# bot15498/Lisec

Hardware: AMD Instinct MI355X
Metric: lyft_samples_per_sec_fwd_bwd (higher is better)
Workload: dtype f32; 1 GPU; Lyft grid 8x200x400x35, U20K synthetic cloud, 1 sample/GPU/step, voxelise+VFE+3xConv3D+RPN fwd+bwd, MSE+MSE, SGD-Nesterov; global_batch=1, parallelism=dp1, launch=step plan (lisec_step_plan_run: 196 recorded launches / event edges per step), voxels=9424

## Files before the change

include/lisec_hip.h:

```cpp
#ifndef LISEC_HIP_H
#define LISEC_HIP_H

#include <stddef.h>
#include <stdint.h>

#ifdef __cplusplus
extern "C" {
#endif

#define LISEC_OK 0
#define LISEC_EINVAL (-1)
#define LISEC_ENOSPC (-2)
#define LISEC_EHIP (-3)

typedef void* lisec_stream_t;

const char* lisec_last_error(void);
int lisec_abi_version(void);
int lisec_device_info(char* name, int cap);

typedef struct {
    double xSize, ySize, zSize;
    int maxVoxelX, maxVoxelY, maxVoxelZ;
    int sampleSize;
// ... 273 lines not shown

int lisec_bn_backward_apply_coef(const float* dA, int da_stride, const float* y, const float* bnstate, long long M, int C,
                                 int relu, const float* coef, float* dy, lisec_stream_t stream);

typedef struct lisec_copy_desc {
    const float* src;
    float* dst;
    int rows, cols;
    long long src_stride, dst_stride;
} lisec_copy_desc;
int lisec_copy2d_batched(const lisec_copy_desc* device_table, int n, lisec_stream_t stream);

int lisec_fold_depth(const float* in, float* out, int D, long long HW, int C, int inverse, const float* mask,
                     lisec_stream_t stream);

int lisec_relu_mask(float* grad, const float* act, long long n, lisec_stream_t stream);

int lisec_colsum(const float* x, int stride, long long M, int C, float* out, void* workspace,
                 size_t workspace_bytes, lisec_stream_t stream);

int lisec_rpn_loss(const float* head, const float* y_cls, const float* y_reg, long long M, int kind,
                   float grad_scale, float* dhead, float* loss_out, void* workspace, size_t workspace_bytes,
                   lisec_stream_t stream);

int lisec_rpn_loss_eval(const float* head, const float* y_cls, const float* y_reg, long long M, int kind, double* acc,
                        void* workspace, size_t workspace_bytes, lisec_stream_t stream);

#define LISEC_LOSS_MAX_METRICS 4
enum {
    LISEC_LOSS_MSE = 0,
    LISEC_LOSS_MAE = 1,
    LISEC_LOSS_MAPE = 2,
    LISEC_LOSS_MSLE = 3,
    LISEC_LOSS_HUBER = 4,
    LISEC_LOSS_LOGCOSH = 5,
    LISEC_LOSS_BCE = 6,
    LISEC_LOSS_POISSON = 7,
    LISEC_LOSS_SIGMOID_CE_CLAMPED = 8,
    LISEC_LOSS_SMOOTH_L1 = 9,
    LISEC_METRIC_BINARY_ACCURACY = 10,
    LISEC_METRIC_CATEGORICAL_ACCURACY = 11
};
typedef struct lisec_loss_term {
    int kind;
    int from_logits;
    float param;
// ... 286 lines not shown
```

lisec_amd/_lib.py:

```python
import ctypes
import os
from ctypes import POINTER, Structure, c_char_p, c_double, c_float, c_int, c_int32, c_size_t, c_void_p

_HERE = os.path.dirname(os.path.abspath(__file__))
LIB_PATH = os.path.join(_HERE, "liblisec_hip.so")


class LisecError(RuntimeError):
    pass


class VoxelCfg(Structure):
    _fields_ = [("xSize", c_double), ("ySize", c_double), ("zSize", c_double),
                ("maxVoxelX", c_int), ("maxVoxelY", c_int), ("maxVoxelZ", c_int),
                ("sampleSize", c_int)]


class VfeParams(Structure):
    _fields_ = [("kernel", c_void_p * 3), ("gamma", c_void_p * 3), ("beta", c_void_p * 3),
                ("moving_mean", c_void_p * 3), ("moving_var", c_void_p * 3)]


class VfeGrads(Structure):
    _fields_ = [("kernel", c_void_p * 3), ("gamma", c_void_p * 3), ("beta", c_void_p * 3)]
# ... 263 lines not shown
    lib.lisec_bn_backward_apply_coef.argtypes = [P, c_int, P, P, LL, c_int, c_int, P, P, P]
    lib.lisec_conv_forward_masked.restype = c_int
    lib.lisec_conv_forward_masked.argtypes = [POINTER(ConvGeom), P, P, P, P, c_int, P, P, P, P, c_size_t, P, P, c_int, P]
    lib.lisec_conv_forward_workspace_bytes.restype = c_size_t
    lib.lisec_conv_forward_workspace_bytes.argtypes = [POINTER(ConvGeom)]
    lib.lisec_conv_forward_rows_workspace_bytes.restype = c_size_t
    lib.lisec_conv_forward_rows_workspace_bytes.argtypes = [POINTER(ConvGeom), c_int]
    lib.lisec_conv_wgrad_workspace_bytes.restype = c_size_t
    lib.lisec_conv_wgrad_workspace_bytes.argtypes = [POINTER(ConvGeom), c_int]
    lib.lisec_conv_wgrad.restype = c_int
    lib.lisec_conv_wgrad.argtypes = [POINTER(ConvGeom), P, P, c_int, P, P, P, c_size_t, c_int, P, P, P, c_int, P]
    lib.lisec_eltwise_workspace_bytes.restype = c_size_t
    lib.lisec_eltwise_workspace_bytes.argtypes = []
    lib.lisec_bn_backward.restype = c_int
    lib.lisec_bn_backward.argtypes = [P, c_int, P, P, LL, c_int, c_int, P, P, P, P, P, c_size_t, P]
    lib.lisec_relu_mask.restype = c_int
    lib.lisec_relu_mask.argtypes = [P, P, LL, P]
    lib.lisec_colsum.restype = c_int
    lib.lisec_colsum.argtypes = [P, c_int, LL, c_int, P, P, c_size_t, P]
    lib.lisec_rpn_loss.restype = c_int
    lib.lisec_rpn_loss.argtypes = [P, P, P, LL, c_int, c_float, P, P, P, c_size_t, P]
    lib.lisec_rpn_loss_eval.restype = c_int
    lib.lisec_rpn_loss_eval.argtypes = [P, P, P, LL, c_int, P, P, c_size_t, P]
    lib.lisec_head_loss.restype = c_int
    lib.lisec_head_loss.argtypes = [POINTER(LossCfg), P, P, P, LL, c_float, P, P, P, P, c_size_t, P]
    lib.lisec_head_loss_eval.restype = c_int
    lib.lisec_head_loss_eval.argtypes = [POINTER(LossCfg), P, P, P, LL, P, P, c_size_t, P]
    lib.lisec_head_loss_workspace_bytes.restype = c_size_t
    lib.lisec_head_loss_workspace_bytes.argtypes = []
    lib.lisec_detection_loss.restype = c_int
    lib.lisec_detection_loss.argtypes = [POINTER(DetectionLossCfg), P, P, P, LL, c_float, P, P, P, P, c_size_t, P]
    lib.lisec_detection_loss_eval.restype = c_int
    lib.lisec_detection_loss_eval.argtypes = [POINTER(DetectionLossCfg), P, P, P, LL, P, P, c_size_t, P]
    lib.lisec_detection_loss_workspace_bytes.restype = c_size_t
    lib.lisec_detection_loss_workspace_bytes.argtypes = []
    lib.lisec_detection_metrics.restype = c_int
    lib.lisec_detection_metrics.argtypes = [POINTER(DetectionMetricsCfg), P, P, P, LL, P, c_int, P, c_size_t, P]
    lib.lisec_detection_metrics_workspace_bytes.restype = c_size_t
    lib.lisec_detection_metrics_workspace_bytes.argtypes = []
    lib.lisec_sgd_nesterov_step.restype = c_int
    lib.lisec_sgd_nesterov_step.argtypes = [P, P, P, LL, c_float, c_float, P]
    lib.lisec_sgd_nesterov_step_dev.restype = c_int
    lib.lisec_sgd_nesterov_step_dev.argtypes = [P, P, P, LL, c_double, c_double, c_float, P, P]
    lib.lisec_sgd_nesterov_step_dev_part.restype = c_int
    lib.lisec_sgd_nesterov_step_dev_part.argtypes = [P, P, P, LL, c_double, c_double, c_float, P, P]
    lib.lisec_sgd_step_dev.restype = c_int
# ... 296 lines not shown
```

lisec_amd/csrc/common.h:

```cpp
#pragma once
#include <hip/hip_runtime.h>
#include <cstdarg>
#include <cstdio>
#include <cstdint>
#include <functional>
#include <tuple>
#include <utility>

#include "../../include/lisec_hip.h"

namespace lisec {

constexpr int kWave = 64;

void set_error(const char* fmt, ...);
const lisec_tuning& tuning();
int cu_count();

#define LISEC_CHECK_ARG(cond, ...)                 \
    do {                                           \
        if (!(cond)) {                             \
            ::lisec::set_error(__VA_ARGS__);       \
            return LISEC_EINVAL;                   \
        }                                          \
// ... 79 lines not shown
__device__ __forceinline__ T wave_sum(T v) {
#pragma unroll
    for (int o = 32; o > 0; o >>= 1) v += __shfl_xor(v, o, 64);
    return v;
}
template <typename T>
__device__ __forceinline__ T wave_max(T v) {
#pragma unroll
    for (int o = 32; o > 0; o >>= 1) {
        T u = __shfl_xor(v, o, 64);
        v = u > v ? u : v;
    }
    return v;
}
template <typename T>
__device__ __forceinline__ T wave_min(T v) {
#pragma unroll
    for (int o = 32; o > 0; o >>= 1) {
        T u = __shfl_xor(v, o, 64);
        v = u < v ? u : v;
    }
    return v;
}
#endif

}
```

lisec_amd/csrc/eltwise.hip:

```cpp
#include "bn.h"

namespace lisec {
namespace {

constexpr int kEwBlocks = 1024;
constexpr int kEwThreads = 256;

template <bool RELU>
__global__ void __launch_bounds__(kEwThreads)
k_bn_bwd_reduce(const float* __restrict__ dA, int da_stride, const float* __restrict__ y,
                const float* __restrict__ st, long long M, int C, double* __restrict__ parts) {
    __shared__ float red[2][kEwThreads][4];
    const int cq = C / 4;
    const int q = threadIdx.x % cq, rsub = threadIdx.x / cq, rows_per_iter = kEwThreads / cq;
    const float4 sc = reinterpret_cast<const float4*>(st)[q];
    const float4 sh = reinterpret_cast<const float4*>(st + C)[q];
    const float4 mu = reinterpret_cast<const float4*>(st + 2 * C)[q];
    const float4 is = reinterpret_cast<const float4*>(st + 3 * C)[q];
    float4 s1 = make_float4(0, 0, 0, 0), s2 = make_float4(0, 0, 0, 0);
    for (long long r = (long long)blockIdx.x * rows_per_iter + rsub; r < M; r += (long long)gridDim.x * rows_per_iter) {
        const float4 g = *reinterpret_cast<const float4*>(dA + r * da_stride + q * 4);
        const float4 v = *reinterpret_cast<const float4*>(y + r * C + q * 4);
#define LISEC_ACC(f)                                                         \
        {                                                                    \
// ... 66 lines not shown
        reinterpret_cast<float4*>(g)[i] = a;
    }
}

__global__ void __launch_bounds__(kEwThreads)
k_colsum(const float* __restrict__ x, int stride, long long M, int C, double* __restrict__ parts) {
    __shared__ float red[kEwThreads];
    const int cols = C < kEwThreads ? C : kEwThreads;
    const int c0 = blockIdx.y * kEwThreads;
    const int c = threadIdx.x % cols, rsub = threadIdx.x / cols, rows_per_iter = kEwThreads / cols;
    float s = 0.f;
    if (rsub < rows_per_iter)
        for (long long r = (long long)blockIdx.x * rows_per_iter + rsub; r < M; r += (long long)gridDim.x * rows_per_iter)
            s += x[r * stride + c0 + c];
    red[threadIdx.x] = rsub < rows_per_iter ? s : 0.f;
    __syncthreads();
    if (threadIdx.x < cols) {
        double a = 0.0;
        for (int k = 0; k < rows_per_iter; ++k) a += (double)red[k * cols + threadIdx.x];
        parts[(size_t)blockIdx.x * C + c0 + threadIdx.x] = a;
    }
}

__global__ void __launch_bounds__(kEwThreads)
k_loss(const float* __restrict__ head, const float* __restrict__ ycls, const float* __restrict__ yreg,
       long long M, int kind, float gscale, float* __restrict__ dhead, double* __restrict__ parts) {
    __shared__ double red[2][kEwThreads / 64];
    double lc = 0.0, lr = 0.0;
    const float wc = gscale / (float)(M * 2), wr = gscale / (float)(M * 14);
    for (long long i = blockIdx.x * (long long)kEwThreads + threadIdx.x; i < M * 16; i += (long long)gridDim.x * kEwThreads) {
        const long long m = i >> 4;
        const int c = (int)(i & 15);
        const float p = head[i];
        float g;
        if (c < 2) {
            const float t = ycls[m * 2 + c];
            if (kind == 0) {
                const float d = p - t;
                lc += (double)d * d;
                g = 2.f * d * wc;
            } else {
                const float tt = fminf(fmaxf(t, 0.f), 1.f);
                lc += (double)(fmaxf(p, 0.f) - p * tt + log1pf(expf(-fabsf(p))));
                g = (1.f / (1.f + expf(-p)) - tt) * wc;
            }
        } else {
            const float t = yreg[m * 14 + (c - 2)];
            const float d = p - t;
            if (kind == 0) {
                lr += (double)d * d;
                g = 2.f * d * wr;
            } else {
                const float ad = fabsf(d);
                lr += (double)(ad < 1.f ? 0.5f * d * d : ad - 0.5f);
                g = (ad < 1.f ? d : (d > 0.f ? 1.f : -1.f)) * wr;
            }
        }
        dhead[i] = g;
    }
    lc = wave_sum(lc); lr = wave_sum(lr);
    if (lane_id() == 0) { red[0][threadIdx.x >> 6] = lc; red[1][threadIdx.x >> 6] = lr; }
    __syncthreads();
    if (threadIdx.x < 2) {
        double a = 0.0;
        for (int k = 0; k < kEwThreads / 64; ++k) a += red[threadIdx.x][k];
        parts[(size_t)blockIdx.x * 2 + threadIdx.x] = a;
    }
}

__global__ void __launch_bounds__(256)
k_loss_finalize(const double* __restrict__ parts, int nparts, double M, float* __restrict__ out) {
    __shared__ double red[2][256];
    double a = 0.0, b = 0.0;
    for (int k = threadIdx.x; k < nparts; k += 256) { a += parts[2 * k]; b += parts[2 * k + 1]; }
    red[0][threadIdx.x] = a; red[1][threadIdx.x] = b;
    __syncthreads();
    for (int o = 128; o > 0; o >>= 1) {
        if ((int)threadIdx.x < o) { red[0][threadIdx.x] += red[0][threadIdx.x + o]; red[1][threadIdx.x] += red[1][threadIdx.x + o]; }
        __syncthreads();
    }
    if (threadIdx.x == 0) {
        a = red[0][0] / (M * 2.0); b = red[1][0] / (M * 14.0);
        out[0] = (float)(a + b); out[1] = (float)a; out[2] = (float)b;
    }
}

__global__ void __launch_bounds__(kEwThreads)
k_loss_eval(const float* __restrict__ head, const float* __restrict__ ycls, const float* __restrict__ yreg,
            long long M, int kind, double* __restrict__ parts) {
    __shared__ double red[2][kEwThreads / 64];
// ... 248 lines not shown
    LISEC_LAUNCH(k_colsum, dim3(nb, slabs), dim3(kEwThreads), 0, st, x, stride, M, C, parts);
    LISEC_LAUNCH_CHECK();
    return launch_reduce_parts(parts, nb, C, 1.0, out, nullptr, st);
}

extern "C" int lisec_rpn_loss(const float* head, const float* y_cls, const float* y_reg, long long M, int kind,
                              float grad_scale, float* dhead, float* loss_out, void* workspace,
                              size_t workspace_bytes, lisec_stream_t stream_) {
    LISEC_CHECK_ARG(head && y_cls && y_reg && dhead && loss_out && workspace && M > 0, "NULL pointer");
    LISEC_CHECK_ARG(kind == 0 || kind == 1, "loss kind must be 0 (mse+mse) or 1 (sigmoid-CE + SmoothL1)");
    if (workspace_bytes < lisec_eltwise_workspace_bytes()) {
        set_error("eltwise workspace too small");
        return LISEC_ENOSPC;
    }
    hipStream_t st = static_cast<hipStream_t>(stream_);
    double* parts = static_cast<double*>(workspace);
    int nb = ew_blocks(M * 16);
    LISEC_LAUNCH(k_loss, dim3(nb), dim3(kEwThreads), 0, st, head, y_cls, y_reg, M, kind, grad_scale, dhead, parts);
    LISEC_LAUNCH(k_loss_finalize, dim3(1), dim3(256), 0, st, parts, nb, (double)M, loss_out);
    LISEC_LAUNCH_CHECK();
    return LISEC_OK;
}

extern "C" int lisec_rpn_loss_eval(const float* head, const float* y_cls, const float* y_reg, long long M, int kind,
                                   double* acc, void* workspace, size_t workspace_bytes, lisec_stream_t stream_) {
    LISEC_CHECK_ARG(head && y_cls && y_reg && acc && workspace && M > 0, "NULL pointer");
    LISEC_CHECK_ARG(kind == 0 || kind == 1, "loss kind must be 0 (mse+mse) or 1 (sigmoid-CE + SmoothL1)");
    if (workspace_bytes < lisec_eltwise_workspace_bytes()) {
        set_error("eltwise workspace too small");
        return LISEC_ENOSPC;
    }
    hipStream_t st = static_cast<hipStream_t>(stream_);
    double* parts = static_cast<double*>(workspace);
    int nb = ew_blocks(M * 16);
    LISEC_LAUNCH(k_loss_eval, dim3(nb), dim3(kEwThreads), 0, st, head, y_cls, y_reg, M, kind, parts);
    LISEC_LAUNCH(k_loss_eval_finalize, dim3(1), dim3(256), 0, st, parts, nb, (double)M, acc);
    LISEC_LAUNCH_CHECK();
    return LISEC_OK;
}

extern "C" int lisec_sgd_nesterov_step(float* theta, const float* grad, float* velocity, long long n,
                                       float lr_t, float momentum, lisec_stream_t stream_) {
    LISEC_CHECK_ARG(theta && grad && velocity && n >= 0 && n % 4 == 0, "sgd: n must be a multiple of 4");
    if (n == 0) return LISEC_OK;
    LISEC_LAUNCH(k_sgd_nesterov, dim3(ew_blocks(n / 4)), dim3(kEwThreads), 0, static_cast<hipStream_t>(stream_),
                       theta, grad, velocity, n / 4, lr_t, momentum);
// ... 41 lines not shown
```

lisec_amd/csrc/head_fused.hip:

```cpp
#include "common.h"

namespace lisec {
namespace {

constexpr int kHeadCols = 16;
constexpr int kMaxUp = 512;

constexpr int kPairs = 16, kSlices = 16;
__global__ void __launch_bounds__(256)
k_head_compose(const float* __restrict__ up_kernel, const float* __restrict__ up_bias, const float* __restrict__ head_w,
               int taps, int Cin, int Cup, long long ts, long long cs, float* __restrict__ Wc,
               const float* __restrict__ bias_in, float* __restrict__ bias_out) {
    __shared__ float sH[kMaxUp * kHeadCols];
    __shared__ float red[kSlices][kPairs][kHeadCols + 1];
    for (int i = threadIdx.x; i < Cup * kHeadCols; i += 256) sH[i] = head_w[i];
    __syncthreads();
    const int pl = threadIdx.x & (kPairs - 1), q = threadIdx.x / kPairs;
    const int idx = blockIdx.x * kPairs + pl;
    const bool live = idx < taps * Cin;
    const int tap = live ? idx / Cin : 0, c = live ? idx - tap * Cin : 0;
    float acc[kHeadCols];
#pragma unroll
    for (int j = 0; j < kHeadCols; ++j) acc[j] = 0.f;
    const float* w = up_kernel + (size_t)tap * Cup * Cin + c;
// ... 75 lines not shown
            for (int j = 0; j < kHeadCols; ++j) red[threadIdx.x][j] += red[threadIdx.x + half][j];
        }
        __syncthreads();
    }
    if (threadIdx.x < kHeadCols)
        d_head_w[(size_t)n * kHeadCols + threadIdx.x] = fmaf(up_bias ? up_bias[n] : 0.f, S[threadIdx.x], red[0][threadIdx.x]);
    if (threadIdx.x == 0 && d_up_bias) {
        float b = 0.f;
        for (int j = 0; j < kHeadCols; ++j) b = fmaf(S[j], head_w[(size_t)n * kHeadCols + j], b);
        d_up_bias[n] = b;
    }
}

struct ShuffleBranches { int n; int ps[4]; float* T[4]; };
template <bool BACKWARD>
__global__ void __launch_bounds__(256)
k_head_shuffle(float* __restrict__ head, int Ho, int Wo, ShuffleBranches br) {
    const int i4 = blockIdx.x * 256 + threadIdx.x;
    if (i4 >= Ho * Wo * (kHeadCols / 4)) return;
    const int m = i4 >> 2, q = i4 & 3;
    const int h = m / Wo, w = m - h * Wo;
    float4 v = *reinterpret_cast<const float4*>(head + (size_t)i4 * 4);
    for (int b = 0; b < br.n; ++b) {
        const int ps = br.ps[b];
        const int pos = (h / ps) * (Wo / ps) + w / ps, tap = (h % ps) * ps + w % ps;
        float4* t = reinterpret_cast<float4*>(br.T[b] + ((size_t)pos * ps * ps + tap) * kHeadCols) + q;
        if (BACKWARD) *t = v;
        else { const float4 u = *t; v.x += u.x; v.y += u.y; v.z += u.z; v.w += u.w; }
    }
    if (!BACKWARD) *reinterpret_cast<float4*>(head + (size_t)i4 * 4) = v;
}

}
}

using namespace lisec;

extern "C" int lisec_head_compose(const float* up_kernel, const float* up_bias, const float* head_w, int taps, int Cin,
                                  int Cup, long long out_tap_stride, long long out_c_stride, float* Wc,
                                  const float* bias_in, float* bias_out, lisec_stream_t stream) {
    LISEC_CHECK_ARG(up_kernel && head_w && Wc && taps > 0 && Cin > 0 && Cup > 0 && Cup <= kMaxUp, "bad compose arguments");
    LISEC_CHECK_ARG(!bias_out || up_bias, "a composite bias needs the branch bias");
    LISEC_LAUNCH(k_head_compose, dim3(cdiv((long long)taps * Cin, kPairs)), dim3(256), 0, static_cast<hipStream_t>(stream),
                       up_kernel, up_bias, head_w, taps, Cin, Cup, out_tap_stride, out_c_stride, Wc, bias_in, bias_out);
    LISEC_LAUNCH_CHECK();
    return LISEC_OK;
}

extern "C" int lisec_head_compose_backward(const float* G, long long g_tap_stride, long long g_c_stride,
// ... 31 lines not shown
```

lisec_amd/network.py:

```python
import ctypes
import json
import os

import numpy as np
import torch

from . import _lib, lr_schedules, ops, optimizer_table
from .losses import DetectionLossSpec, LossSpec
from .params import DECONVS, MID, RPN_BLOCKS, ParamStore, fold_depth
from .vfe import VFEStack


LEGACY_LOSS_KINDS = {"mse": 0, "smoothl1_ce": 1}


def loss_acc_len(loss):
    if isinstance(loss, LossSpec):
        return 4 + loss.n_metrics
    if isinstance(loss, DetectionLossSpec):
        return 4 + 2 * loss.n_metrics
    LEGACY_LOSS_KINDS[loss]
    return 4


# ... 185 lines not shown
    def deconv_wgrad(self, L):
        net, a, p, G = self.net, self.net.act, self.net.params, self.net.grad
        c = L["conv"]
        if net.compose_head:
            b, (ts, cs) = L["slot"], L["wc_strides"]
            ops.conv_wgrad(c.g, a[L["src"]], self.branch_dy(L), L["G"], net.wgrad_ws, in_bn=net.bnstate[c.in_bn],
                           flags=ops.IN_RELU)
            ops.head_compose_backward(L["G"], ts, cs, p.view(L["up_kernel"]), p.view(L["up_bias"]),
                                      net.head_w[256 * b:256 * (b + 1)],
                                      net.head_db, L["k"] * L["k"], L["cin"], 256, p.grad_view(G, L["up_kernel"]),
                                      p.grad_view(G, L["up_bias"]), net.head_dw[256 * b:256 * (b + 1)])
            self.branches_left -= 1
            if self.branches_left == 0:
                net._head_split.run()
            return
        dy = self.branch_dy(L)
        if "wgeom" in L:
            ops.conv_wgrad(L["wgeom"], dy, a[L["src"]], p.grad_view(G, c.wname), net.wgrad_ws,
                           flags=ops.DY_RELU, dy_bn=net.bnstate[c.in_bn])
        else:
            ops.conv_wgrad(c.g, a[L["src"]], dy, p.grad_view(G, c.wname), net.wgrad_ws,
                           in_bn=net.bnstate[c.in_bn], flags=ops.IN_RELU, transpose_out=True)

    def heads(self):
        net, q, a, d = self.net, self.q, self.net.act, self.net.dact
        M = net.Ho * net.Wo
        if net.compose_head:
            net._dshuffle.run(d["head"], backward=True)
            q.defer(lambda: ops.colsum(d["head"], 16, M, 16, net.head_db, ws_tag="side"))
            return

        def head_leaves():
            ops.conv_wgrad(net.head_geom, a["concat"], d["head"], net.head_dw, net.wgrad_ws)
            ops.colsum(d["head"], 16, M, 16, net.head_db, ws_tag="side")
            net._head_split.run()

        def concat_leaves():
            ops.colsum(d["concat"], 768, M, 768, net.up_db, ws_tag="side")
            net._up_bias_split.run()

        q.run(head_leaves)
        ops.conv_forward(net.head_dgeom, d["head"], net.packed_t["head"][0], d["concat"])
        q.run(concat_leaves)

    def early_branches(self):
        net, q = self.net, self.q
        for L in net.layers:
            if L["kind"] == "deconv" and L["slot"] < len(DECONVS) - 1:
                ev = net._event("bwd_branch%d" % L["slot"])

                def branch(L=L, ev=ev):
# ... 244 lines not shown
        self.head_w = torch.empty(768, 16, dtype=f32, device=dev)
        self.head_b = torch.empty(16, dtype=f32, device=dev)
        self.fused_bias = torch.empty(16, dtype=f32, device=dev)
        if self.compose_head:
            self._shuffle = ops.HeadShuffle(Ho, Wo, [(L["T"], L["s"]) for L in self.layers
                                                     if L["kind"] == "deconv" and L["T"] is not None])
        self.parts = torch.empty(max_parts, dtype=torch.float64, device=dev)
        self._sinks, self._bsinks = {}, {}
        self.side = torch.cuda.Stream(device=dev, priority=0)
        self.side_queue = _SideQueue(self, None, self.side)

        self._tail_ok = {}
        self._loss_descs = {}
        self._early = None
        self.dense_dw_slabs = {}
        self._fwd_events = {}
        self._pack_pending = self._late_pending = False
        self._pack_done = self._pack_late = None
        self._packed_version = -1
        self.params_version = 0
        self.state_version = 0
        self._folded = {}
        self._train_ready = False
        self._iter_dev = torch.zeros(2, dtype=torch.int64, device=dev)
        self._iterations = 0
        self.momentum_cache = torch.ones(1, dtype=torch.float32, device=dev)
        self._lr_dev = torch.zeros(ctypes.sizeof(_lib.LrSchedule), dtype=torch.uint8, device=dev)
        self._lr_host = None
        self.loss_out = torch.zeros(3, dtype=f32, device=dev)
        self.metric_out = torch.zeros(2 * _lib.LOSS_MAX_METRICS, dtype=f32, device=dev)
        self.loss_counts = torch.zeros(2, dtype=torch.int64, device=dev)
        self.metric_pairs = torch.zeros(2 * _lib.DET_MAX_METRICS, dtype=torch.float64, device=dev)

    @property
    def iterations(self):
        return self._iterations

    @iterations.setter
    def iterations(self, k):
        self._iterations = int(k)
        self._iter_dev.copy_(torch.tensor([int(k), 0], dtype=torch.int64))

    def _pack_all(self, after_main=None):
        if self._packed_version == (self.params_version, self.params.version):
            if after_main is not None:
                after_main()
# ... 111 lines not shown
    def _record(ev, stream):
        ev.record(stream.cuda_stream)

    @staticmethod
    def _wait(ev, stream):
        ev.wait(stream.cuda_stream)

    def _mark(self, name):
        marks = getattr(self, "phase_marks", None)
        if marks is None:
            return
        ev = marks.get(name)
        if ev is None:
            ev = marks[name] = _lib.DeviceEvent(timing=True)
        ev.record(_lib.current_stream())

    def dense_grid(self, rewrite=True):
        if "grid" not in self.act:
            self.act["grid"] = torch.empty(self.grid_shape, dtype=torch.float32, device=self.device)
        if rewrite:
            self.vfe.rewrite_grid(self.act["grid"])
        return self.act["grid"]

    def forward(self, sample, training=False):
        if sample.grid_shape != (self.D, self.H, self.W) or sample.cfg.sampleSize != self.T:
            raise ValueError("voxel sample does not match the model's grid")
        if training:
            self._refuse_bf16_training()
        prev_pin = _lib.pin_stream(torch.cuda.current_stream().cuda_stream)
        try:
            return self._forward(sample, training)
        finally:
            _lib.pin_stream(prev_pin)

    def _forward(self, sample, training):
        self._mark("step:begin")
        pending = self._pack_pending
        if pending and (self._packed_version != (self.params_version, self.params.version)):
            self._wait(self._pack_late, torch.cuda.current_stream())
            self._pack_pending = pending = False
            self._late_pending = False
        if not pending:
            self._pack_all()
        a = self.act
        use_field = self._used_field = self.field_conv and sample.cap <= self.field_max_voxels
        if use_field:
            first = self.layers[0]["conv"]
            need = ops.conv_field_forward_workspace_bytes(first.g, sample.cap)
            if self.field_ws is None or self.field_ws.numel() < need:
                self.field_ws = torch.empty(need, dtype=torch.uint8, device=self.device)
                _lib.bump_alloc_generation()
            self.vfe.forward(sample, training, dense=False)
        else:
            self.vfe.forward(sample, training, out=self.dense_grid(rewrite=False))
        self._mark("step:vfe done")
        if pending:
            self._wait(self._pack_done, torch.cuda.current_stream())
            self._pack_pending = False
# ... 28 lines not shown
                    dst = a["head"] if L["T"] is None else L["T"]

                    def run(ws_tag, c=c, L=L, dst=dst):
                        ops.conv_forward(c.g, a[L["src"]], self.packed[c.name], dst,
                                         bias=self.fused_bias if L["T"] is None else None, in_bn=self.bnstate[c.in_bn],
                                         flags=ops.IN_RELU, ws_tag=ws_tag)
                else:
                    def run(ws_tag, L=L, b=b):
                        self._run_conv(L["conv"], a[L["src"]], a["concat"][:, :, 256 * b:], training, ws_tag=ws_tag)
                if b < len(DECONVS) - 1:
                    q.mark_fork(self._event("fwd_fork%d" % b))
                    q.run(lambda: run("side"))
                    side_used = True
                else:
                    if self._late_pending:
                        self._wait(self._pack_late, torch.cuda.current_stream())
                        self._late_pending = False
                    run("main")
        if self._late_pending:
            self._wait(self._pack_late, torch.cuda.current_stream())
            self._late_pending = False
        if side_used:
            q.join(self._event("fwd_join"))
        if self.compose_head:
            self._shuffle.run(a["head"])
        else:
            ops.conv_forward(self.head_geom, a["concat"], self.packed["head"], a["head"], bias=self.head_b)
        head = a["head"]
        return head[None, :, :, :2], head[None, :, :, 2:]

    def _refuse_bf16_training(self):
        if self.compute_dtype != "float32":
            raise NotImplementedError("a bfloat16-compute network serves inference only: training in mixed precision is not "
                                      "implemented (build the network with compute_dtype='float32')")

    def _prepare_training(self):
        if self._train_ready:
            return
        dev, f32 = self.device, torch.float32
        p = self.params
        self.grad = torch.zeros_like(p.theta)
        self.velocity = torch.zeros_like(p.theta)
        self._slots = {"velocity": self.velocity}
        self.dact = {}
        for name, t in self.act.items():
            if name.endswith(".u") or name in ("concat", "head", "fold") or ".y" in name:
                self.dact[name] = torch.empty_like(t)
        self.packed_t = {}
        self.dgeom = {}
        ws_bytes = ops.wgrad_workspace_bytes(self.head_geom)
# ... 31 lines not shown
                self.dgeom[c.name] = ops.geom(1, (g.Do, g.Ho, g.Wo), (g.Di, g.Hi, g.Wi), (g.KD, g.KH, g.KW),
                                              (g.sd, g.sh, g.sw), (g.pd, g.ph, g.pw), g.Cout, g.Cin)
                self.packed_t[c.name] = (torch.empty(ops.packed_floats(ntaps, g.Cout, g.Cin), dtype=f32, device=dev),
                                         (ntaps, g.Cout, g.Cin, g.Cin * g.Cout, 1, g.Cout))
            if "dense" in L:
                d = L["dense"]
                ws_bytes = max(ws_bytes, ops.wgrad_workspace_bytes(d.g))
                self.dgeom[d.name] = d.g
                self.packed_t[d.name] = (torch.empty(ops.packed_floats(1, 64, 64), dtype=f32, device=dev),
                                         (1, 64, 64, 0, 1, 64))
                self.dact[L["name"] + ".z"] = torch.empty_like(self.act[L["name"] + ".y"])
        first = self.layers[0]["conv"]
        self.mid1_S = torch.empty(27 * 64, dtype=f32, device=dev)
        self.g_all = torch.empty(64, dtype=f32, device=dev)
        self.tapsum_ws = torch.empty(ops.tap_sums_workspace_bytes(first.g), dtype=torch.uint8, device=dev)
        self.dout_rows = None
        self.rows_queue = torch.zeros(2, dtype=torch.int32, device=dev)
        self.head_dgeom = ops.geom(0, (1, Ho, Wo), (1, Ho, Wo), (1, 1, 1), (1, 1, 1), (0, 0, 0), 16, 768)
        if not self.compose_head:
            self.packed_t["head"] = (torch.empty(ops.packed_floats(1, 16, 768), dtype=f32, device=dev), None)
        else:
            self._dshuffle = ops.HeadShuffle(Ho, Wo, [(L["dT"], L["s"]) for L in self.layers
                                                      if L["kind"] == "deconv" and L["dT"] is not None])
        self.head_dw = torch.empty(768, 16, dtype=f32, device=dev)
        self.up_db = torch.empty(768, dtype=f32, device=dev)
        self.bn_of, self.consumers = {}, {}
        nparts = 1
        for L in self.layers:
            self.consumers[L["src"]] = self.consumers.get(L["src"], 0) + 1
            if L["kind"] == "conv":
                self.bn_of[L["dst"]] = (L["conv"].bn, L["conv"].g.Cout)
        for L in self.layers:
            if L["src"] in self.bn_of:
                nparts = max(nparts, ops.num_mblocks_bwd(self.dgeom[L["conv"].name]) * 2 * self.bn_of[L["src"]][1])
            if "dense" in L:
                nparts = max(nparts, ops.num_mblocks_bwd(self.dgeom[L["dense"].name]) * 2 * 64)
        self.bparts = torch.empty(nparts, dtype=torch.float64, device=dev)
        self.head_db = torch.empty(16, dtype=f32, device=dev)
        G = self.grad
        self._head_split = ops.CopyTable([(self.head_dw[:, :2], p.grad_view(G, "cls.kernel")[0, 0]),
                                          (self.head_dw[:, 2:], p.grad_view(G, "reg.kernel")[0, 0]),
                                          (self.head_db[:2], p.grad_view(G, "cls.bias")),
                                          (self.head_db[2:], p.grad_view(G, "reg.bias"))], self.device)
        if not self.compose_head:
            self._up_bias_split = ops.CopyTable(
                [(self.up_db[256 * L["slot"]:256 * (L["slot"] + 1)], p.grad_view(G, L["conv"].bias))
# ... 65 lines not shown
        finally:
            _lib.pin_stream(prev_pin)

    def _loss_descriptor(self, spec):
        if spec not in self._loss_descs:
            self._loss_descs[spec] = spec.descriptor()
        return self._loss_descs[spec]

    def _metrics_descriptor(self, spec):
        key = ("metrics", spec)
        if key not in self._loss_descs:
            self._loss_descs[key] = spec.metrics_descriptor()
        return self._loss_descs[key]

    def step_metrics(self, loss):
        if isinstance(loss, LossSpec) and loss.n_metrics:
            return self.metric_out[:loss.n_metrics]
        if isinstance(loss, DetectionLossSpec) and loss.n_metrics:
            return self.metric_pairs[:2 * loss.n_metrics]
        return None

    def _loss_backward(self, loss, y_cls, y_reg, grad_scale):
        head, dhead, M = self.act["head"], self.dact["head"], self.Ho * self.Wo
        if isinstance(loss, LossSpec):
            ops.head_loss(self._loss_descriptor(loss), head, y_cls, y_reg, M, dhead, self.loss_out, self.metric_out,
                          grad_scale=grad_scale)
        elif isinstance(loss, DetectionLossSpec):
            ops.detection_loss(self._loss_descriptor(loss), head, y_cls, y_reg, M, dhead, self.loss_out, self.loss_counts,
                               grad_scale=grad_scale)
            if loss.n_metrics:
                ops.detection_metrics(self._metrics_descriptor(loss), head, y_cls, y_reg, M, self.metric_pairs)
        else:
            ops.rpn_loss(head, y_cls, y_reg, M, LEGACY_LOSS_KINDS[loss], dhead, self.loss_out, grad_scale=grad_scale)

    def loss_eval(self, loss, y_cls, y_reg, acc):
        head, M = self.act["head"], self.Ho * self.Wo
        if isinstance(loss, LossSpec):
            ops.head_loss_eval(self._loss_descriptor(loss), head, y_cls, y_reg, M, acc)
        elif isinstance(loss, DetectionLossSpec):
            ops.detection_loss_eval(self._loss_descriptor(loss), head, y_cls, y_reg, M, acc)
            if loss.n_metrics:
                ops.detection_metrics(self._metrics_descriptor(loss), head, y_cls, y_reg, M, acc[4:], accumulate=True)
        else:
            ops.rpn_loss_eval(head, y_cls, y_reg, M, LEGACY_LOSS_KINDS[loss], acc)

    def _tail_supported(self, c, dst_name):
        ok = self._tail_ok.get(c.name)
        if ok is None:
            n = dst_name[:-2]
            Ln = {L["name"]: L for L in self.layers}.get(n)
            ok = False
            if Ln is not None and "dense" in Ln and self.dgeom[c.name].Cout == 64:
                cn, dn = Ln["conv"], Ln["dense"]
                try:
                    ops.conv_plan(self.dgeom[c.name], out_mask=self.act[dst_name],
                                  bwd=(self.act[n + ".y"], self.bnstate[cn.bn], False), sink=self._bwd_sink(cn.bn, 64, cn.M),
# ... 3 lines not shown
                    ok = False
            self._tail_ok[c.name] = ok
        return ok

    def _size_backward_scratch(self, sample):
        first = self.layers[0]["conv"]
        need = ops.wgrad_workspace_bytes(self.dgeom[first.name], max(sample.cap, 1))
        if need > self.wgrad_ws.numel() or self.dout_rows is None or self.dout_rows.shape[0] < sample.cap + 1:
            torch.cuda.synchronize()
            if need > self.wgrad_ws.numel():
                self.wgrad_ws = torch.zeros(need, dtype=torch.uint8, device=self.device)
            self.dout_rows = torch.empty((sample.cap + 1, 64), dtype=torch.float32, device=self.device)
            _lib.bump_alloc_generation()

    def _backward(self, y_cls, y_reg, loss, grad_scale, rpn_grads_ready, side_filler=None):
        self._prepare_training()
        self._pack_all_t()
        sample = self.vfe._sample
        self._size_backward_scratch(sample)
        q = self.side_queue
        q.begin(torch.cuda.current_stream())
        bp = _BackwardPass(self, q, sample, rpn_grads_ready, side_filler)
        self._mark("bwd:start")
        self._loss_backward(loss, y_cls, y_reg, grad_scale)
        bp.heads()
        bp.early_branches()
        step = {"deconv": bp.deconv, "conv": bp.conv, "mid": bp.mid}
        for L in reversed(self.layers):
            self._mark("bwd:before " + L["name"])
            step[L["kind"]](L)
        bp.finish()
        return self.loss_out

    def slot(self, name):
        self._prepare_training()
        t = self._slots.get(name)
        if t is None:
            if name not in self.SLOT_NAMES:
                raise KeyError(f"unknown optimizer slot {name!r}")
            t = self._slots[name] = torch.zeros_like(self.params.theta)
            torch.cuda.synchronize(self.device)
        return t

    SLOT_NAMES = optimizer_table.SLOT_NAMES

    def slots(self):
        self._prepare_training()
        return dict(self._slots)
# ... 54 lines not shown
                self._pack_all_t()
            finally:
                _lib.pin_stream(pin)
            self._record(self._pack_late, self.side)
            self._pack_pending = True
            self._late_pending = True

    def _arm_repack(self):
        self._pack_pending = self._late_pending = False
        self._pack_all()
        self._pack_all_t()
        self._record(self._pack_done, torch.cuda.current_stream())
        self._record(self._pack_late, torch.cuda.current_stream())
        self._pack_pending = self._late_pending = True

    def _replayed(self):
        self._iterations += 1
        self.params_version += 1
        self.state_version += 1
        self._packed_version = self._packed_t_version = (self.params_version, self.params.version)
        self._pack_pending = self._late_pending = True

    def train_step(self, sample, y_cls, y_reg, loss="mse", allreduce=None, opt=None, side_filler=None):
        self.forward(sample, training=True)
        if allreduce is not None and hasattr(allreduce, "start_tail"):
            self.backward(y_cls, y_reg, loss=loss, side_filler=side_filler,
                          rpn_grads_ready=lambda lo, hi: allreduce.start_tail(self.grad, lo, hi))
            allreduce.finish(self.grad)
        elif allreduce is not None:
            self.backward(y_cls, y_reg, loss=loss, side_filler=side_filler)
            allreduce(self.grad)
        else:
            self.backward(y_cls, y_reg, loss=loss, side_filler=side_filler,
                          rpn_grads_ready=lambda lo, hi: self.early_update(lo, hi, opt=opt))
        self.apply_gradients(opt=opt)
        return self.loss_out


class StalePlanError(RuntimeError):
    """A recorded step plan holds raw addresses of buffers that an eager call has since reallocated."""


class _StepPlans:

    PAD = 1.0e6

    def __init__(self, net, voxelizer, capacity, nbuf, dtype, loss):
# ... 237 lines not shown
```

lisec_amd/ops.py:

```python
import ctypes
import math

import torch

from . import _lib
from ._lib import ConvGeom

IN_RELU, OUT_RELU, ACCUMULATE, DY_RELU, SMALL_TILE, TAG_ROOFLINE = 1, 2, 4, 8, 16, 32


def geom(mode, in_dims, out_dims, kernel, stride, pad, cin, cout, in_stride=None, out_stride=None, ps=0,
         ps_channels=0):
    g = ConvGeom()
    g.mode = mode
    g.Di, g.Hi, g.Wi = in_dims
    g.Do, g.Ho, g.Wo = out_dims
    g.KD, g.KH, g.KW = kernel
    g.sd, g.sh, g.sw = stride
    g.pd, g.ph, g.pw = pad
    g.Cin, g.Cout = cin, cout
    g.in_stride = in_stride if in_stride is not None else cin
    g.out_stride = out_stride if out_stride is not None else cout
    g.ps, g.ps_channels = ps, ps_channels
    return g
# ... 567 lines not shown


def head_compose_backward(G, tap_stride, c_stride, up_kernel, up_bias, head_w, S, taps, cin, cup, d_up_kernel, d_up_bias,
                          d_head_w):
    _lib.check(_lib.load().lisec_head_compose_backward(_lib.ptr(G), tap_stride, c_stride, _lib.ptr(up_kernel),
                                                       _lib.ptr(up_bias), _lib.ptr(head_w), _lib.ptr(S), taps, cin, cup,
                                                       _lib.ptr(d_up_kernel),
                                                       _lib.ptr(d_up_bias), _lib.ptr(d_head_w), _lib.current_stream()))


class HeadShuffle:

    def __init__(self, Ho, Wo, branches):
        self.Ho, self.Wo, self.n = Ho, Wo, len(branches)
        self.keep = [t for t, _ in branches]
        self.T = (ctypes.c_void_p * self.n)(*[t.data_ptr() for t, _ in branches])
        self.ps = (ctypes.c_int * self.n)(*[p for _, p in branches])

    def run(self, head, backward=False):
        _lib.check(_lib.load().lisec_head_shuffle(_lib.ptr(head), self.Ho, self.Wo, self.n, self.T, self.ps,
                                                  1 if backward else 0, _lib.current_stream()))


def augment_params(rot_box=math.pi / 10, sigma=(1.0, 1.0, 0.0), scale=(0.95, 1.05), rot_global=math.pi / 4, attempts=10):
    p = _lib.AugmentParams()
    p.rot_box, p.rot_global, p.attempts = float(rot_box), float(rot_global), int(attempts)
    p.scale_lo, p.scale_hi = float(scale[0]), float(scale[1])
    for i in range(3):
        p.sigma[i] = float(sigma[i])
    return p


def _int32_count(n_boxes):
    if n_boxes.dtype != torch.int32 or n_boxes.numel() != 1 or not n_boxes.is_cuda:
        raise ValueError("a device-side box count is one int32 on the device")
    return _lib.ptr(n_boxes)


def augment_draw(boxes, params, seed=0, item=0, epoch=0, n_boxes=None):
    B, dev = int(boxes.shape[0]), boxes.device
    new = torch.empty if n_boxes is None else torch.zeros
    transforms = new((B, 4), dtype=torch.float64, device=dev)
    glob = torch.empty(2, dtype=torch.float64, device=dev)
    boxes_out = new((B, 7), dtype=torch.float64, device=dev)
    attempt = new(B, dtype=torch.int32, device=dev)
    draws = new(4 + 8 * B, dtype=torch.int32, device=dev)
# ... 76 lines not shown
```

Baseline: 287.7 samples/s.

## Fuse head branch join, RPN loss and gradient scatter into one kernel

During training the forward pass now skips the separate head shuffle join. A new kernel sums the deconv branch taps into the head, computes the MSE/CE loss and gradient, and scatters dhead back into each branch's dT in one pass. The loss reduction finalize is deferred onto the side queue. This removes the forward shuffle, the separate loss, and the backward shuffle launches and their memory passes, at the cost of scalar (non-float4) strided branch accesses and more complex control flow between forward and backward.

```diff
diff --git a/include/lisec_hip.h b/include/lisec_hip.h
--- a/include/lisec_hip.h
+++ b/include/lisec_hip.h
@@ -319,6 +319,12 @@
 int lisec_rpn_loss(const float* head, const float* y_cls, const float* y_reg, long long M, int kind,
                    float grad_scale, float* dhead, float* loss_out, void* workspace, size_t workspace_bytes,
                    lisec_stream_t stream);
+
+size_t lisec_rpn_loss_parts(long long M);
+int lisec_head_join_loss(float* head, int Ho, int Wo, int n_branches, const float* const* T, float* const* dT,
+                         const int* ps, const float* y_cls, const float* y_reg, int kind, float grad_scale, float* dhead,
+                         double* parts, size_t parts_len, lisec_stream_t stream);
+int lisec_rpn_loss_finalize(const double* parts, long long M, float* loss_out, lisec_stream_t stream);
 
 int lisec_rpn_loss_eval(const float* head, const float* y_cls, const float* y_reg, long long M, int kind, double* acc,
                         void* workspace, size_t workspace_bytes, lisec_stream_t stream);
diff --git a/lisec_amd/_lib.py b/lisec_amd/_lib.py
--- a/lisec_amd/_lib.py
+++ b/lisec_amd/_lib.py
@@ -309,6 +309,13 @@
     lib.lisec_rpn_loss.argtypes = [P, P, P, LL, c_int, c_float, P, P, P, c_size_t, P]
     lib.lisec_rpn_loss_eval.restype = c_int
     lib.lisec_rpn_loss_eval.argtypes = [P, P, P, LL, c_int, P, P, c_size_t, P]
+    lib.lisec_rpn_loss_parts.restype = c_size_t
+    lib.lisec_rpn_loss_parts.argtypes = [LL]
+    lib.lisec_head_join_loss.restype = c_int
+    lib.lisec_head_join_loss.argtypes = [P, c_int, c_int, c_int, POINTER(c_void_p), POINTER(c_void_p), POINTER(c_int), P, P,
+                                         c_int, c_float, P, P, c_size_t, P]
+    lib.lisec_rpn_loss_finalize.restype = c_int
+    lib.lisec_rpn_loss_finalize.argtypes = [P, LL, P, P]
     lib.lisec_head_loss.restype = c_int
     lib.lisec_head_loss.argtypes = [POINTER(LossCfg), P, P, P, LL, c_float, P, P, P, P, c_size_t, P]
     lib.lisec_head_loss_eval.restype = c_int
diff --git a/lisec_amd/csrc/common.h b/lisec_amd/csrc/common.h
--- a/lisec_amd/csrc/common.h
+++ b/lisec_amd/csrc/common.h
@@ -125,6 +125,11 @@
     }
     return v;
 }
+
+__device__ __forceinline__ size_t shuffle_cell(int h, int w, int Wo, int ps) {
+    const int pos = (h / ps) * (Wo / ps) + w / ps, tap = (h % ps) * ps + w % ps;
+    return ((size_t)pos * ps * ps + tap) * 16;
+}
 #endif
 
 }
diff --git a/lisec_amd/csrc/eltwise.hip b/lisec_amd/csrc/eltwise.hip
--- a/lisec_amd/csrc/eltwise.hip
+++ b/lisec_amd/csrc/eltwise.hip
@@ -112,42 +112,38 @@
     }
 }
 
-__global__ void __launch_bounds__(kEwThreads)
-k_loss(const float* __restrict__ head, const float* __restrict__ ycls, const float* __restrict__ yreg,
-       long long M, int kind, float gscale, float* __restrict__ dhead, double* __restrict__ parts) {
+__device__ __forceinline__ float loss_element(float p, long long m, int c, const float* __restrict__ ycls,
+                                              const float* __restrict__ yreg, int kind, float wc, float wr, double& lc,
+                                              double& lr) {
+    float g;
+    if (c < 2) {
+        const float t = ycls[m * 2 + c];
+        if (kind == 0) {
+            const float d = p - t;
+            lc += (double)d * d;
+            g = 2.f * d * wc;
+        } else {
+            const float tt = fminf(fmaxf(t, 0.f), 1.f);
+            lc += (double)(fmaxf(p, 0.f) - p * tt + log1pf(expf(-fabsf(p))));
+            g = (1.f / (1.f + expf(-p)) - tt) * wc;
+        }
+    } else {
+        const float t = yreg[m * 14 + (c - 2)];
+        const float d = p - t;
+        if (kind == 0) {
+            lr += (double)d * d;
+            g = 2.f * d * wr;
+        } else {
+            const float ad = fabsf(d);
+            lr += (double)(ad < 1.f ? 0.5f * d * d : ad - 0.5f);
+            g = (ad < 1.f ? d : (d > 0.f ? 1.f : -1.f)) * wr;
+        }
+    }
+    return g;
+}
+
+__device__ __forceinline__ void loss_block_partials(double lc, double lr, double* __restrict__ parts) {
     __shared__ double red[2][kEwThreads / 64];
-    double lc = 0.0, lr = 0.0;
-    const float wc = gscale / (float)(M * 2), wr = gscale / (float)(M * 14);
-    for (long long i = blockIdx.x * (long long)kEwThreads + threadIdx.x; i < M * 16; i += (long long)gridDim.x * kEwThreads) {
-        const long long m = i >> 4;
-        const int c = (int)(i & 15);
-        const float p = head[i];
-        float g;
-        if (c < 2) {
-            const float t = ycls[m * 2 + c];
-            if (kind == 0) {
-                const float d = p - t;
-                lc += (double)d * d;
-                g = 2.f * d * wc;
-            } else {
-                const float tt = fminf(fmaxf(t, 0.f), 1.f);
-                lc += (double)(fmaxf(p, 0.f) - p * tt + log1pf(expf(-fabsf(p))));
-                g = (1.f / (1.f + expf(-p)) - tt) * wc;
-            }
-        } else {
-            const float t = yreg[m * 14 + (c - 2)];
-            const float d = p - t;
-            if (kind == 0) {
-                lr += (double)d * d;
-                g = 2.f * d * wr;
-            } else {
-                const float ad = fabsf(d);
-                lr += (double)(ad < 1.f ? 0.5f * d * d : ad - 0.5f);
-                g = (ad < 1.f ? d : (d > 0.f ? 1.f : -1.f)) * wr;
-            }
-        }
-        dhead[i] = g;
-    }
     lc = wave_sum(lc); lr = wave_sum(lr);
     if (lane_id() == 0) { red[0][threadIdx.x >> 6] = lc; red[1][threadIdx.x >> 6] = lr; }
     __syncthreads();
@@ -156,6 +152,45 @@
         for (int k = 0; k < kEwThreads / 64; ++k) a += red[threadIdx.x][k];
         parts[(size_t)blockIdx.x * 2 + threadIdx.x] = a;
     }
+}
+
+__global__ void __launch_bounds__(kEwThreads)
+k_loss(const float* __restrict__ head, const float* __restrict__ ycls, const float* __restrict__ yreg,
+       long long M, int kind, float gscale, float* __restrict__ dhead, double* __restrict__ parts) {
+    double lc = 0.0, lr = 0.0;
+    const float wc = gscale / (float)(M * 2), wr = gscale / (float)(M * 14);
+    for (long long i = blockIdx.x * (long long)kEwThreads + threadIdx.x; i < M * 16; i += (long long)gridDim.x * kEwThreads)
+        dhead[i] = loss_element(head[i], i >> 4, (int)(i & 15), ycls, yreg, kind, wc, wr, lc, lr);
+    loss_block_partials(lc, lr, parts);
+}
+
+struct JoinBranches { int n; int ps[4]; const float* T[4]; float* dT[4]; };
+__global__ void __launch_bounds__(kEwThreads)
+k_head_join_loss(float* __restrict__ head, int Ho, int Wo, JoinBranches br, const float* __restrict__ ycls,
+                 const float* __restrict__ yreg, int kind, float gscale, float* __restrict__ dhead,
+                 double* __restrict__ parts) {
+    double lc = 0.0, lr = 0.0;
+    const long long M = (long long)Ho * Wo;
+    const float wc = gscale / (float)(M * 2), wr = gscale / (float)(M * 14);
+    for (long long i = blockIdx.x * (long long)kEwThreads + threadIdx.x; i < M * 16; i += (long long)gridDim.x * kEwThreads) {
+        const long long m = i >> 4;
+        const int c = (int)(i & 15), h = (int)(m / Wo), w = (int)(m - (long long)h * Wo);
+        size_t at[4];
+        float p = head[i];
+#pragma unroll
+        for (int b = 0; b < 4; ++b)
+            if (b < br.n) {
+                at[b] = shuffle_cell(h, w, Wo, br.ps[b]) + c;
+                p += br.T[b][at[b]];
+            }
+        head[i] = p;
+        const float g = loss_element(p, m, c, ycls, yreg, kind, wc, wr, lc, lr);
+        dhead[i] = g;
+#pragma unroll
+        for (int b = 0; b < 4; ++b)
+            if (b < br.n) br.dT[b][at[b]] = g;
+    }
+    loss_block_partials(lc, lr, parts);
 }
 
 __global__ void __launch_bounds__(256)
@@ -450,6 +485,40 @@
     return LISEC_OK;
 }
 
+extern "C" size_t lisec_rpn_loss_parts(long long M) { return M > 0 ? (size_t)2 * ew_blocks(M * 16) : 0; }
+
+extern "C" int lisec_head_join_loss(float* head, int Ho, int Wo, int n_branches, const float* const* T, float* const* dT,
+                                    const int* ps, const float* y_cls, const float* y_reg, int kind, float grad_scale,
+                                    float* dhead, double* parts, size_t parts_len, lisec_stream_t stream_) {
+    LISEC_CHECK_ARG(head && y_cls && y_reg && dhead && parts && Ho > 0 && Wo > 0, "NULL pointer");
+    LISEC_CHECK_ARG(n_branches >= 0 && n_branches <= 4 && (n_branches == 0 || (T && dT && ps)), "bad branch arguments");
+    LISEC_CHECK_ARG(kind == 0 || kind == 1, "loss kind must be 0 (mse+mse) or 1 (sigmoid-CE + SmoothL1)");
+    JoinBranches br;
+    br.n = n_branches;
+    for (int b = 0; b < n_branches; ++b) {
+        LISEC_CHECK_ARG(T[b] && dT[b] && ps[b] >= 1 && Ho % ps[b] == 0 && Wo % ps[b] == 0,
+                        "branch %d: stride must divide the map", b);
+        br.ps[b] = ps[b]; br.T[b] = T[b]; br.dT[b] = dT[b];
+    }
+    const long long M = (long long)Ho * Wo;
+    if (parts_len < lisec_rpn_loss_parts(M)) {
+        set_error("loss partials too small");
+        return LISEC_ENOSPC;
+    }
+    LISEC_LAUNCH(k_head_join_loss, dim3(ew_blocks(M * 16)), dim3(kEwThreads), 0, static_cast<hipStream_t>(stream_), head, Ho,
+                       Wo, br, y_cls, y_reg, kind, grad_scale, dhead, parts);
+    LISEC_LAUNCH_CHECK();
+    return LISEC_OK;
+}
+
+extern "C" int lisec_rpn_loss_finalize(const double* parts, long long M, float* loss_out, lisec_stream_t stream_) {
+    LISEC_CHECK_ARG(parts && loss_out && M > 0, "NULL pointer");
+    LISEC_LAUNCH(k_loss_finalize, dim3(1), dim3(256), 0, static_cast<hipStream_t>(stream_), parts, ew_blocks(M * 16),
+                       (double)M, loss_out);
+    LISEC_LAUNCH_CHECK();
+    return LISEC_OK;
+}
+
 extern "C" int lisec_rpn_loss_eval(const float* head, const float* y_cls, const float* y_reg, long long M, int kind,
                                    double* acc, void* workspace, size_t workspace_bytes, lisec_stream_t stream_) {
     LISEC_CHECK_ARG(head && y_cls && y_reg && acc && workspace && M > 0, "NULL pointer");
diff --git a/lisec_amd/csrc/head_fused.hip b/lisec_amd/csrc/head_fused.hip
--- a/lisec_amd/csrc/head_fused.hip
+++ b/lisec_amd/csrc/head_fused.hip
@@ -121,9 +121,7 @@
     const int h = m / Wo, w = m - h * Wo;
     float4 v = *reinterpret_cast<const float4*>(head + (size_t)i4 * 4);
     for (int b = 0; b < br.n; ++b) {
-        const int ps = br.ps[b];
-        const int pos = (h / ps) * (Wo / ps) + w / ps, tap = (h % ps) * ps + w % ps;
-        float4* t = reinterpret_cast<float4*>(br.T[b] + ((size_t)pos * ps * ps + tap) * kHeadCols) + q;
+        float4* t = reinterpret_cast<float4*>(br.T[b] + shuffle_cell(h, w, Wo, br.ps[b])) + q;
         if (BACKWARD) *t = v;
         else { const float4 u = *t; v.x += u.x; v.y += u.y; v.z += u.z; v.w += u.w; }
     }
diff --git a/lisec_amd/network.py b/lisec_amd/network.py
--- a/lisec_amd/network.py
+++ b/lisec_amd/network.py
@@ -231,11 +231,14 @@
             ops.conv_wgrad(c.g, a[L["src"]], dy, p.grad_view(G, c.wname), net.wgrad_ws,
                            in_bn=net.bnstate[c.in_bn], flags=ops.IN_RELU, transpose_out=True)
 
-    def heads(self):
+    def heads(self, scattered=False):
         net, q, a, d = self.net, self.q, self.net.act, self.net.dact
         M = net.Ho * net.Wo
         if net.compose_head:
-            net._dshuffle.run(d["head"], backward=True)
+            if scattered:
+                q.defer(lambda: net._join_loss.finalize(net.loss_out))
+            else:
+                net._dshuffle.run(d["head"], backward=True)
             q.defer(lambda: ops.colsum(d["head"], 16, M, 16, net.head_db, ws_tag="side"))
             return
 
@@ -526,6 +529,7 @@
         self.state_version = 0
         self._folded = {}
         self._train_ready = False
+        self._join_pending = False
         self._iter_dev = torch.zeros(2, dtype=torch.int64, device=dev)
         self._iterations = 0
         self.momentum_cache = torch.ones(1, dtype=torch.float32, device=dev)
@@ -683,18 +687,18 @@
             self.vfe.rewrite_grid(self.act["grid"])
         return self.act["grid"]
 
-    def forward(self, sample, training=False):
+    def forward(self, sample, training=False, join=True):
         if sample.grid_shape != (self.D, self.H, self.W) or sample.cfg.sampleSize != self.T:
             raise ValueError("voxel sample does not match the model's grid")
         if training:
             self._refuse_bf16_training()
         prev_pin = _lib.pin_stream(torch.cuda.current_stream().cuda_stream)
         try:
-            return self._forward(sample, training)
+            return self._forward(sample, training, join)
         finally:
             _lib.pin_stream(prev_pin)
 
-    def _forward(self, sample, training):
+    def _forward(self, sample, training, join=True):
         self._mark("step:begin")
         pending = self._pack_pending
         if pending and (self._packed_version != (self.params_version, self.params.version)):
@@ -769,10 +773,11 @@
             self._late_pending = False
         if side_used:
             q.join(self._event("fwd_join"))
-        if self.compose_head:
+        self._join_pending = self.compose_head and not join
+        if not self.compose_head:
+            ops.conv_forward(self.head_geom, a["concat"], self.packed["head"], a["head"], bias=self.head_b)
+        elif join:
             self._shuffle.run(a["head"])
-        else:
-            ops.conv_forward(self.head_geom, a["concat"], self.packed["head"], a["head"], bias=self.head_b)
         head = a["head"]
         return head[None, :, :, :2], head[None, :, :, 2:]
 
@@ -850,6 +855,8 @@
         else:
             self._dshuffle = ops.HeadShuffle(Ho, Wo, [(L["dT"], L["s"]) for L in self.layers
                                                       if L["kind"] == "deconv" and L["dT"] is not None])
+            self._join_loss = ops.HeadJoinLoss(Ho, Wo, [(L["T"], L["dT"], L["s"]) for L in self.layers
+                                                        if L["kind"] == "deconv" and L["dT"] is not None], dev)
         self.head_dw = torch.empty(768, 16, dtype=f32, device=dev)
         self.up_db = torch.empty(768, dtype=f32, device=dev)
         self.bn_of, self.consumers = {}, {}
@@ -961,6 +968,12 @@
 
     def _loss_backward(self, loss, y_cls, y_reg, grad_scale):
         head, dhead, M = self.act["head"], self.dact["head"], self.Ho * self.Wo
+        pending, self._join_pending = self._join_pending, False
+        if pending and isinstance(loss, str):
+            self._join_loss.run(head, y_cls, y_reg, LEGACY_LOSS_KINDS[loss], dhead, grad_scale=grad_scale)
+            return True
+        if pending:
+            self._shuffle.run(head)
         if isinstance(loss, LossSpec):
             ops.head_loss(self._loss_descriptor(loss), head, y_cls, y_reg, M, dhead, self.loss_out, self.metric_out,
                           grad_scale=grad_scale)
@@ -971,6 +984,7 @@
                 ops.detection_metrics(self._metrics_descriptor(loss), head, y_cls, y_reg, M, self.metric_pairs)
         else:
             ops.rpn_loss(head, y_cls, y_reg, M, LEGACY_LOSS_KINDS[loss], dhead, self.loss_out, grad_scale=grad_scale)
+        return False
 
     def loss_eval(self, loss, y_cls, y_reg, acc):
         head, M = self.act["head"], self.Ho * self.Wo
@@ -1020,8 +1034,7 @@
         q.begin(torch.cuda.current_stream())
         bp = _BackwardPass(self, q, sample, rpn_grads_ready, side_filler)
         self._mark("bwd:start")
-        self._loss_backward(loss, y_cls, y_reg, grad_scale)
-        bp.heads()
+        bp.heads(scattered=self._loss_backward(loss, y_cls, y_reg, grad_scale))
         bp.early_branches()
         step = {"deconv": bp.deconv, "conv": bp.conv, "mid": bp.mid}
         for L in reversed(self.layers):
@@ -1122,7 +1135,7 @@
         self._pack_pending = self._late_pending = True
 
     def train_step(self, sample, y_cls, y_reg, loss="mse", allreduce=None, opt=None, side_filler=None):
-        self.forward(sample, training=True)
+        self.forward(sample, training=True, join=False)
         if allreduce is not None and hasattr(allreduce, "start_tail"):
             self.backward(y_cls, y_reg, loss=loss, side_filler=side_filler,
                           rpn_grads_ready=lambda lo, hi: allreduce.start_tail(self.grad, lo, hi))
diff --git a/lisec_amd/ops.py b/lisec_amd/ops.py
--- a/lisec_amd/ops.py
+++ b/lisec_amd/ops.py
@@ -613,6 +613,26 @@
                                                   1 if backward else 0, _lib.current_stream()))
 
 
+class HeadJoinLoss:
+
+    def __init__(self, Ho, Wo, branches, device):
+        self.Ho, self.Wo, self.n = Ho, Wo, len(branches)
+        self.keep = [t for b in branches for t in b[:2]]
+        self.T = (ctypes.c_void_p * max(self.n, 1))(*[t.data_ptr() for t, _, _ in branches])
+        self.dT = (ctypes.c_void_p * max(self.n, 1))(*[t.data_ptr() for _, t, _ in branches])
+        self.ps = (ctypes.c_int * max(self.n, 1))(*[p for _, _, p in branches])
+        self.parts = torch.empty(_lib.load().lisec_rpn_loss_parts(Ho * Wo), dtype=torch.float64, device=device)
+
+    def run(self, head, y_cls, y_reg, kind, dhead, grad_scale=1.0):
+        _lib.check(_lib.load().lisec_head_join_loss(_lib.ptr(head), self.Ho, self.Wo, self.n, self.T, self.dT, self.ps,
+                                                    _lib.ptr(y_cls), _lib.ptr(y_reg), kind, grad_scale, _lib.ptr(dhead),
+                                                    _lib.ptr(self.parts), self.parts.numel(), _lib.current_stream()))
+
+    def finalize(self, loss_out):
+        _lib.check(_lib.load().lisec_rpn_loss_finalize(_lib.ptr(self.parts), self.Ho * self.Wo, _lib.ptr(loss_out),
+                                                       _lib.current_stream()))
+
+
 def augment_params(rot_box=math.pi / 10, sigma=(1.0, 1.0, 0.0), scale=(0.95, 1.05), rot_global=math.pi / 4, attempts=10):
     p = _lib.AugmentParams()
     p.rot_box, p.rot_global, p.attempts = float(rot_box), float(rot_global), int(attempts)
```

Measured after the change: 288.5 samples/s (median of 6 runs). About the same (+0.3%).
